# waiwera/waiwera

Measured on AMD Instinct MI355X. Metric: Newton steps/sec, 10M-cell eos_we (BCSR SpMV GB/s in roofline), higher is better.
Workload: dtype f64

## Files before the change

waiwera_amd/csrc/context.hpp:

```cpp
#pragma once
#include <hip/hip_runtime.h>
#include <string>
#include <type_traits>
#include <vector>
#include "../../include/waiwera_hip.h"
#include "colour_order.hpp"
#include "coupling_batch.hpp"
#include "devbuf.hpp"
#include "ilu_schedule.hpp"
#include "mesh_pattern.hpp"
#include "network_pass.hpp"
#include "network_wave.hpp"
#include "physics.hip.h"
#include "tile_schedule.hpp"

namespace wai {

__host__ __device__ __forceinline__ size_t ell_ld(size_t n) {
  size_t ld = (n + 511) & ~(size_t)511;
  if ((ld & 262143) == 0) ld += 512;
  return ld;
}
__host__ __device__ __forceinline__ size_t ell_rows(int bs, size_t n) {
  if (bs >= 3) return ell_ld(n);
  return n;
}
__host__ __device__ __forceinline__ size_t ell_ix1(int bs, size_t n, int r, int k, size_t i) {
  if (bs >= 3) return ((i >> 6) * (size_t)(bs * bs) + (size_t)(r * bs + k)) * 64 + (i & 63);
  return ((size_t)r * n + i) * bs + k;
}
__host__ __device__ __forceinline__ size_t ell_ix(int bs, size_t n, int s, int r, int k, size_t i) {
  if (bs >= 3) {
    const size_t bb = (size_t)(bs * bs);
    return (size_t)(s >> 3) * 8 * bb * ell_ld(n) + ((((i >> 6) << 3) + (size_t)(s & 7)) * bb + (size_t)(r * bs + k)) * 64 + (i & 63);
  }
  return ((size_t)(s * bs + r) * n + i) * bs + k;
}
__host__ __device__ __forceinline__ size_t ell_size(int bs, size_t n, int W) {
  if (bs >= 3) return (size_t)((W + 7) / 8) * 8 * bs * bs * ell_ld(n);
  return (size_t)W * bs * bs * ell_rows(bs, n);
}

enum KClass { KC_EOS = 0, KC_RESIDUAL = 1, KC_JACOBIAN = 2, KC_SPMV = 3, KC_PC_APPLY = 4,
              KC_PC_SETUP = 5, KC_VECTOR = 6, KC_TRANSITIONS = 7, KC_COUNT = 8 };

enum { S_RHO = 0, S_RHOOLD = 1, S_ALPHA = 2, S_OMEGA = 3, S_BETA = 4, S_D1 = 5, S_D2 = 6,
       S_DP2 = 7, S_RHONEW = 8, S_W2 = 9, S_BREAK = 15, S_H = 16 };

enum PcDot { PC_DOT_NONE = 0, PC_DOT_ZA = 1, PC_DOT_XZ = 2, PC_DOT_ZZ = 3, PC_DOT_MERGED = 4 };
static_assert(S_D2 == S_D1 + 1 && S_DP2 == S_D1 + 2 && S_RHONEW == S_D1 + 3 && S_W2 == S_D1 + 4,
              "the merged reductions' slots S_D1 .. S_W2 are consecutive: a reduction addresses them as slot0 + index");
__host__ __device__ constexpr int pc_dot_slot0(int mode) { return mode == PC_DOT_ZZ ? S_DP2 : S_D1; }
__host__ __device__ constexpr int pc_dot_nslots(int mode) {
  return mode == PC_DOT_MERGED ? 5 : (mode == PC_DOT_XZ ? 2 : (mode == PC_DOT_NONE ? 0 : 1));
}

struct Comm;

struct DeviceMesh {
  int n_owned = 0, n_halo = 0, n_bc = 0, n_prim = 0, n_local = 0, n_faces = 0, max_deg = 0;
  DevBuf<double> rock;
  DevBuf<double> vol;
  DevBuf<double> fgeom;
  DevBuf<int> fdir;
  DevBuf<int> adj_face;
  DevBuf<int> adj_other;
  DevBuf<int> adj_blk;
  DevBuf<int> adj_tblk;
  DevBuf<int> diag_blk;
  DevBuf<int> cell_src;
  DevBuf<int> face_cells;
};

struct Sources {
  int n = 0;
  DevBuf<int> cell, comp, pcomp, next;
  DevBuf<double> rate, enth;
  DevBuf<SrcCtl> ctl;
  DevBuf<double> net;
};

struct NetNode { double rate = 0, enth = 0, wrate = 0, wenth = 0, srate = 0, senth = 0; };
struct NetRef { int kind = 0, index = -1; };
struct NetGroup {
  std::vector<NetRef> in;
  int scaling = 0;
  int n_limit = 0, limit_type[3] = {0, 0, 0};
  double limit[3] = {0, 0, 0};
  SrcCtl sep{};
  NetNode node;
};
struct NetOutput {
  int flow = 1;
  NetRef out;
  double rate = -1.0, proportion = -1.0, enthalpy = -1.0;
  NetNode node;
};
struct NetReinjector {
  NetRef in;
  std::vector<NetOutput> out;
  NetRef overflow;
  NetNode node;
  double in_w = 0, in_wh = 0, in_s = 0, in_sh = 0;
  double out_w = 0, out_s = 0;
  NetNode over;
  bool fed = false;
};
struct Network {
  bool on = false;
  std::vector<NetGroup> groups;
  std::vector<NetReinjector> reinjectors;
  std::vector<int> reinj_order;
  std::vector<int> rate_specified, enth_specified;
  std::vector<NetNode> src;
  std::vector<double> h_enth0, h_raw, out_rate, out_enth;
  std::vector<char> is_out;
  std::vector<SrcCtl> h_ctl;
  DevBuf<double> d_raw;
  std::vector<int> gidx;
  int n_global = 0;
  DevBuf<double> d_all;
  std::vector<double> h_loc, l_net, l_enth;
  std::vector<int> h_cell;
  bool coupling = true;
  bool cp_in_pc = true;
  bool cp_valid = false;
  std::vector<int> cp_cells;
  std::vector<double> h_cp_val;
  bool cp_span = false;
  int cp_m = 0, cp_j0 = 0;
  std::vector<int> cp_owner;
  DevBuf<int> d_cp_cells;
  DevBuf<double> d_cp_val, d_cp_f, d_cp_g;
  DevBuf<double> d_cp_x;
  NetFlatHost flat;
  bool flat_fits = false, flat_dirty = true;
  DevBuf<int> d_flat_iw;
  NetWaveHost wave;
  bool wave_built = false, wave_ok = false;
  std::string wave_err;
  DevBuf<int> d_wave_ww;
  DevBuf<double> d_flat_dw;
  DevBuf<double> d_state;
  bool state_on_device = false;
  bool enth_stale = false;
  DevBuf<double> d_cp_yh;
  DevBuf<int> d_cp_flag;
  bool cp_on_device = false;
  DevBuf<double> d_cb_scratch;
  long long cb_doubles = 0;
};

struct Bcsr {
  int n = 0, ncols = 0, nnzb = 0, bs = 0, W = 0;
  int* col = nullptr;
  double* val = nullptr;
  int* rowptr = nullptr;
  int dg = 0;
  double* fdg = nullptr;
};
struct Pattern {
  int n = 0, ncols = 0, nnzb = 0, W = 0;
  DevBuf<int> col;
  DevBuf<int> rowptr;
  std::vector<int> h_rowptr, h_colidx;
};

struct LinSys;
struct TileTables : TileFacts {
  DevBuf<int> tile_ptr;
  DevBuf<int> tile_nin;
  DevBuf<int> ord_f, ord_b;
  DevBuf<int> row_lev;
  void clear() {
    static_cast<TileFacts&>(*this) = TileFacts();
    tile_ptr.reset(); tile_nin.reset(); ord_f.reset(); ord_b.reset(); row_lev.reset();
  }
};
struct IluSchedule : ScheduleFacts {
  DevBuf<int> sub_ptr;
  DevBuf<int> sub_nlev;
  DevBuf<int> sub_split;
  DevBuf<int> row_info;
  DevBuf<unsigned long long> row_infow;
  DevBuf<double> fval;
  DevBuf<double> dinv;
  DevBuf<int> row_uoff;
  DevBuf<int> row_tslot;
  DevBuf<int> sub_int;
  DevBuf<int> sub_bnd;
  DevBuf<int> sub_order;
  DevBuf<int> row_uoffw;
  DevBuf<unsigned short> col16;
  DevBuf<int> sub_seg;
  DevBuf<int> t_info, t_uoff;
  DevBuf<unsigned short> t_col16;
  DevBuf<int> sub_desc;
  DevBuf<int> pack_tab[3];
  DevBuf<int> ord_f;
  DevBuf<int> ord_b;
  TileTables tiles;
  const LinSys* owner = nullptr;
};
struct ColourSchedule : ColourFacts {
  bool built = false;
  bool fused = false;
  DevBuf<int> sub_ptr;
  DevBuf<int> sub_ncol;
  DevBuf<int> rows;
  DevBuf<unsigned long long> slots;
  DevBuf<int> counts;
};
inline int pc_threads(const IluSchedule& s) { return ((s.max_rows + 63) / 64) * 64; }

template <class F>
int with_bs(int bs, F&& f) {
  switch (bs) {
    case 1: f(std::integral_constant<int, 1>{}); return 0;
    case 2: f(std::integral_constant<int, 2>{}); return 0;
    case 3: f(std::integral_constant<int, 3>{}); return 0;
    case 4: f(std::integral_constant<int, 4>{}); return 0;
    default: return -1;
  }
}
template <class F>
void with_flag(bool flag, F&& f) {
  if (flag) f(std::true_type{});
  else f(std::false_type{});
}
template <class F>
int with_eos(int kind, F&& f) {
  switch (kind) {
    case EOS_W: f(std::integral_constant<int, EOS_W>{}); return 0;
    case EOS_WE: f(std::integral_constant<int, EOS_WE>{}); return 0;
    case EOS_WCE: f(std::integral_constant<int, EOS_WCE>{}); return 0;
    case EOS_WSE: f(std::integral_constant<int, EOS_WSE>{}); return 0;
    case EOS_WAE: f(std::integral_constant<int, EOS_WAE>{}); return 0;
    case EOS_WSCE: f(std::integral_constant<int, EOS_WSCE>{}); return 0;
    case EOS_WSAE: f(std::integral_constant<int, EOS_WSAE>{}); return 0;
    default: return -1;
  }
}
struct EosTraits { int np, df, nmob; bool salt; };
inline int eos_traits(int kind, EosTraits& t) {
  return with_eos(kind, [&](auto k) {
    constexpr int K = decltype(k)::value;
    t = EosTraits{EosT<K>::np, EosT<K>::df, EosT<K>::nmob, is_salt<K>};
  });
}

struct AsmSystem {
  int overlap = -1;
  int levels = 0;
  bool sublu = false;
  bool fused = false, fuse_asked = false;
  int n_ext = 0;
  Bcsr E;
  DevBuf<int> E_col;
  DevBuf<double> E_val;
  IluSchedule sched;
  DevBuf<int> ext_row;
  DevBuf<int> gmap;
  DevBuf<double> r_ext;
  bool with_net = false;
  int n_net = 0;
  DevBuf<int> net_pos;
  DevBuf<int> net_pair;
  bool cross = false;
  DevBuf<double> hval;
  DevBuf<double> r_full;
};

struct ResForm {
  int method = 0;
  double dt = 0.0, ratio = 0.0;
  const double* last = nullptr;
  const double* last2 = nullptr;
};

constexpr int MAX_TRACERS = 8;
constexpr int POST_OFF = 64;
constexpr unsigned long long POST_KEY = 0x5bd1e995a5a5c3c3ull;
struct Tracers {
  int nt = 0;
  int phase[MAX_TRACERS] = {0};
  double decay[MAX_TRACERS] = {0}, activation[MAX_TRACERS] = {0}, diffusion[MAX_TRACERS] = {0};
  double* bc = nullptr;
  double* inj = nullptr;
  double* rhsb = nullptr;
  int mode = 0;
  long long n_sweeps = 0;
  unsigned char kernarg_tail[136] = {0};
};
static_assert(sizeof(Tracers) == 408, "Tracers is a kernel argument (k_tracer_assemble_all, k_tracer_lhs): its size is part of their argument layout");
static_assert(std::is_trivially_copyable<Tracers>::value, "a kernel argument holds views, never an owner");

struct TracerForm {
  int method, it, nt, phase;
  double dt, ratio, decay, activation, diffusion;
};
static_assert(std::is_trivially_copyable<TracerForm>::value && std::is_trivially_copyable<ResForm>::value &&
              std::is_trivially_copyable<EosParams>::value, "a kernel argument holds views, never an owner");

constexpr int FIN_MAXF = 64;
struct Fin {
  int count = 0;
  int nb = 0;
  int nf = 1;
  double* part2 = nullptr;
  int slot0 = 0, nslots = 0;
  int phase = -1;
  int seq = 0;
  double* scal = nullptr;
  double* post = nullptr;
};
static_assert(std::is_trivially_copyable<Fin>::value, "a kernel argument holds views, never an owner");

struct Krylov {
  double* d_post = nullptr;
  int seq = 0;
  long long n_launch = 0, n_copy = 0;
  DevBuf<double> partials;
  DevBuf<double> partials2;
  DevBuf<unsigned> started;
  bool alpha_pending = false;
  int nb_max = 0;
  DevBuf<double> scal;
  PinnedBuf<double> h_scal;
  int nblocks = 0;
  int nb_pc = 0;
};

struct KrylovVecs {
  DevBuf<double> R, RP, P, V, S, T, tmp, X_own;
  double* X = nullptr;
  DevBuf<double> bl;
  DevBuf<double> basis;
  int basis_m = 0;
};

struct KspOpts {
  int type = WAI_KSP_BCGS, restart = 30, max_its = 10000;
  double rtol = 1.e-5, atol = 1.e-50;
};
struct PcOpts {
  int type = WAI_AUX_PC_FOLLOW, asm_overlap = 1, ilu_levels = 0, sub = WAI_SUB_ILU;
};

struct LinSys {
  Bcsr A;
  DevBuf<double> val, fdg;
  KspOpts ksp;
  PcOpts pc;
  int n = 0, nl = 0;
  KrylovVecs* kv = nullptr;
  AsmSystem as;
  bool net_blocks = false;
};

struct Gather {
  DevBuf<double> in;
  DevBuf<double> send;
  DevBuf<double> recv;
  DevBuf<double> out;
  DevBuf<double> counts;
  DevBuf<int> idx;
  DevBuf<int> claim;
  DevBuf<int> flag;
  size_t n_in = 0, n_send = 0, n_recv = 0, n_out = 0, n_counts = 0, n_idx = 0, n_claim = 0;
};

}

namespace wai {
struct LuBlocks {
  DevBuf<double> inv;
  DevBuf<size_t> inv_ptr;
  std::vector<size_t> h_inv_ptr;
  size_t total = 0;
  int bs = 0;
};
int launch_lu_apply(wai_ctx* c, int bs, const double* r, double* z);

struct Handles {
  hipStream_t stream = nullptr;
  Comm* comm = nullptr;
  hipEvent_t ev_scal = nullptr;
  hipStream_t comm_stream = nullptr;
  hipEvent_t ev_pack = nullptr, ev_halo = nullptr;
  hipEvent_t ev0 = nullptr, ev1 = nullptr, pev0 = nullptr, pev1 = nullptr;
  Handles() = default;
  Handles(const Handles&) = delete;
  ~Handles();
};
}

struct wai_ctx : wai::Handles {
  int device = 0;
  int n_cu = 256;
  size_t lds_per_block = 64 * 1024;
  int kind = 0, np = 0, df = 0, nmob = 0;
  bool salt = false;
  wai::EosParams ep{};
  wai_solver_opts opts{};
  int sub_pc = WAI_SUB_ILU;
  int net_pass = WAI_NETWORK_PASS_HOST;
  int net_walk = WAI_NETWORK_WALK_LANE;
  int net_wave_attr = 0;
  long long net_passes = 0, net_waits = 0;
  int cp_build = WAI_COUPLING_BUILD_COLUMNS;
  long long cp_launches = 0, cp_columns = 0, cp_chunks = 0;
  int pc_ordering = WAI_PC_ORDER_NATURAL;
  wai::ColourSchedule colour;
  std::vector<int> pc_tiles;
  wai::DeviceMesh mesh;
  wai::Sources src;
  wai::Network net;
  std::vector<int> src_gidx;
  int src_nglobal = 0;
  wai::Pattern pat;
  wai::LinSys flow, aux, coupled;
  wai::KrylovVecs kv, kv_coupled;
  wai::IluSchedule ilu;
  wai::LuBlocks lu;
  wai::Krylov ks;
  wai::Tracers tr;
  wai::Gather gat;
  wai::DevBuf<double> tr_bc, tr_inj, tr_rhsb;
  wai::DevBuf<double> flu, flu_last_iter, flu_last_step, flu_pert;
  wai::DevBuf<double> hstep;
  wai::DevBuf<double> w_y, w_yold, w_delta, w_f, w_lhs, w_a, w_b, w_c;
  wai::DevBuf<int> d_flags;
  wai::PinnedBuf<int> h_flags;
  wai::DevBuf<double> d_red;
  wai::PinnedBuf<double> h_red;
  wai::DevBuf<double> stage[4];
  size_t stage_len = 0;
  struct EnvSw {
    bool fin_separate = false; bool no_col16 = false; bool scalar_kernels = false; bool iluk_level_path = false;
    bool asm_unfused = false; bool no_desc_share = false; bool no_pack = false;
    bool colour_sweeps = false;
    int park_stage = -1;
  } env;
  int test_drop_wait = 0;
  int n_nbr = 0;
  std::vector<int> nbr_rank, send_ptr, recv_ptr;
  wai::DevBuf<int> d_send_idx; wai::DevBuf<double> d_sendbuf, d_recvbuf;
  int send_total = 0, max_dof_buf = 0;
  double fnorm0 = 0.0;
  int method = 0;
  double ratio = 0.0;
  wai::DevBuf<double> w_lhs2;
  int scheme = 0, taken = 0;
  double dt_last = 0.0;
  wai::DevBuf<double> w_hist;
  wai::DevBuf<double> w_hist_prev;
  double dt_last_prev = 0.0;
  bool can_reject = false;
  bool prof_on = false;
  bool last_iter_partial = false;
  double prof_ms[wai::KC_COUNT] = {0};
  long long prof_n[wai::KC_COUNT] = {0};
  std::string err;
  bool bc_set = false;
  int dbg = 0;
};

namespace wai {
int launch_eos(wai_ctx* c, const double* y, int first, int count, bool perturbed);
int launch_residual(wai_ctx* c, double dt, const double* lhs_old, double* f, double* lhs_out,
                    double* rhs_out, const int* only = nullptr, int n_only = 0);
int launch_jacobian(wai_ctx* c, double dt, const double* lhs_old);
int launch_transitions(wai_ctx* c, const double* y_old, double* search, double* y);
int launch_tracer_assemble(wai_ctx* c, const TracerForm& tf, const double* alx_last,
                           const double* alx_last2, double* b);
int launch_tracer_assemble_all(wai_ctx* c, int method, double dt, double ratio, const double* alx_last,
                               const double* alx_last2, double* b);
int launch_tracer_lhs(wai_ctx* c, double* Al);
int launch_separator(wai_ctx* c, double pressure, double* out);
int launch_face_fluxes(wai_ctx* c, const int* face_cells, double* out);
int launch_source_rates(wai_ctx* c, double* out, bool raw = false);
int launch_network_pass(wai_ctx* c, const double* raw, double* net, double* enth, double* state_out, bool wave);
int net_wave_allow_lds(wai_ctx* c, const void* kernel, int bit, size_t* bytes);
int launch_cp_perturb(wai_ctx* c, double* p, double* yh);
int launch_cp_restore(wai_ctx* c, double* p, const double* yh);
int launch_cp_diff(wai_ctx* c, int ml, int m, int bs, int j, int k, const double* g, const double* yh, double* val, int* flag);
int launch_coupling_batch(wai_ctx* c, const CouplingBatch& b, int col0, int ncol, double dt, const double* y, const double* lhs_old,
                          long long* launches, bool wave);
int launch_tracer_pick(wai_ctx* c, const double* X, int it, double* x);
int launch_tracer_put(wai_ctx* c, const double* x, int it, double* X);
int launch_tracer_alx(wai_ctx* c, const double* X, double* alx);
int launch_max_scaled(wai_ctx* c, const double* v, const double* scale, double tol, double* val,
                      int* idx);
int launch_fluid_aos(wai_ctx* c, const double* flu_soa, double* out_aos);
int launch_region_get(wai_ctx* c, double* out);
int launch_region_set(wai_ctx* c, const double* in, int first, int count);

int launch_spmv(wai_ctx* c, const Bcsr& M, const double* x, double* y);
int launch_ilu_factor_on(wai_ctx* c, const Bcsr& M, IluSchedule& s);
int launch_pc_on(wai_ctx* c, const Bcsr& M, const IluSchedule& s, bool spmv, const double* in, double* z,
                 int dot_mode, const double* aux, const int* list = nullptr, int nrun = 0, const Fin* fin = nullptr,
                 const double* in2 = nullptr, const Bcsr* F = nullptr, const int* row_map = nullptr);
int pc_kernel_kind(const wai_ctx* c, const Bcsr& M, const IluSchedule& s);
bool pc_axpy_capable(const wai_ctx* c, const Bcsr& M);
bool pc_axpy_default(const wai_ctx* c, const Bcsr& M);
int launch_big_solve(wai_ctx* c, const Bcsr& M, const IluSchedule& s, double* z);
int launch_colour_factor(wai_ctx* c, const Bcsr& M, const ColourSchedule& k, IluSchedule& s);
int launch_colour_solve(wai_ctx* c, const Bcsr& M, const ColourSchedule& k, const IluSchedule& s, double* z);
bool pc_colour_serves(const wai_ctx* c, const Bcsr& M, const ColourSchedule& k, bool one_rank);
int launch_pc_colour(wai_ctx* c, const Bcsr& M, const ColourSchedule& k, const IluSchedule& s, bool spmv, const double* in, double* z,
                     int dot_mode, const double* aux, const Fin* fin = nullptr);
int launch_sublu_solve(wai_ctx* c, const Bcsr& M, const IluSchedule& s, double* z);
bool sublu_vector_in_lds(const IluSchedule& s, int bs);
int launch_asm_gather_matrix(wai_ctx* c, const Bcsr& M, const AsmSystem& a);
int launch_pack_rows(wai_ctx* c, const Bcsr& M);
int launch_unpack_rows(wai_ctx* c, const Bcsr& M, const AsmSystem& a);
int launch_asm_gather(wai_ctx* c, const AsmSystem& a, const double* r);
int launch_asm_scatter(wai_ctx* c, const AsmSystem& a, double* z);
int vec_dots(wai_ctx* c, const double* a1, const double* b1, int slot1, const double* a2, const double* b2,
             int slot2, int n);
int launch_pc(wai_ctx* c, const Bcsr& M, bool spmv, const double* in, double* z, int dot_mode, const double* aux,
              const int* list = nullptr, int nrun = 0, const Fin* fin = nullptr, const double* in2 = nullptr);
Fin make_fin(wai_ctx* c, int slot0, int nslots, int phase, bool post = false);
inline Fin make_fin_dots(wai_ctx* c, int dot_mode, int phase, bool post = false) {
  return make_fin(c, pc_dot_slot0(dot_mode), pc_dot_nslots(dot_mode), phase, post);
}
int launch_ell_to_bcsr(wai_ctx* c, const Bcsr& M, double* bcsr);
int launch_dg_spmv(wai_ctx* c, const Bcsr& M, const double* x, double* y);
int launch_dg_factor(wai_ctx* c, const Bcsr& M, IluSchedule& s);
int launch_dg_pc(wai_ctx* c, const Bcsr& M, const IluSchedule& s, bool spmv, const double* in, double* z, const int* list, int nrun);
int launch_dg_big_solve(wai_ctx* c, const Bcsr& M, const IluSchedule& s, double* z);
int launch_dg_to_bcsr(wai_ctx* c, const Bcsr& M, double* bcsr);
int launch_bcsr_to_ell(wai_ctx* c, const double* bcsr, const Bcsr& M);
int vec_finalize(wai_ctx* c, int nb, int slot0, int nslots, int phase);
int vec_dot(wai_ctx* c, const double* a, const double* b, int n, int slot);
int partials_clear(wai_ctx* c, int slot0, int nslots);
int vec_copy(wai_ctx* c, double* dst, const double* src, size_t n);
int vec_zero(wai_ctx* c, double* dst, size_t n);
int vec_waxpy(wai_ctx* c, double* w, double alpha, const double* x, const double* y, int n);
int bcgs_scalars(wai_ctx* c, int phase, bool post = false);
int bcgs_update_xrp_derive(wai_ctx* c, const KrylovVecs& k, int n);
int bcgs_post(wai_ctx* c, int seq);
void read_env(wai_ctx* c);
int test_drop_partials(wai_ctx* c, int n);
int bcgs_update_p(wai_ctx* c, const KrylovVecs& k, int n);
int bcgs_update_s(wai_ctx* c, const KrylovVecs& k, int n);
int bcgs_update_xr(wai_ctx* c, const KrylovVecs& k, int n, bool dots = true, int fin_phase = -2, bool post = false);
int bcgs_update_xrp(wai_ctx* c, const KrylovVecs& k, int n);
int pack_halo_axpy(wai_ctx* c, const double* a, const double* b, int dof, hipStream_t stream = nullptr);
int gmres_mdot(wai_ctx* c, const double* basis, size_t ld, int n, const double* w, int k);
int gmres_maxpy_norm(wai_ctx* c, const double* basis, size_t ld, int n, double* w, int k);
int gmres_scale_to(wai_ctx* c, double* dst, const double* src, int slot_norm2, int n);
int gmres_update_x(wai_ctx* c, const double* basis, size_t ld, int n, double* x, const double* ycoef_host, int k);
int pack_halo(wai_ctx* c, const double* vec, int dof, hipStream_t stream = nullptr);
int unpack_halo(wai_ctx* c, double* vec, int dof, hipStream_t stream = nullptr);
}
```

waiwera_amd/csrc/linalg_device.hip.h:

```cpp
#pragma once
#include "context.hpp"

namespace wai {

constexpr int TPB = 256;

template <int CTRL, int ROW_MASK, int BANK_MASK>
__device__ __forceinline__ double dpp_add(double v) {
  const int lo = __builtin_amdgcn_update_dpp(0, __double2loint(v), CTRL, ROW_MASK, BANK_MASK, false);
  const int hi = __builtin_amdgcn_update_dpp(0, __double2hiint(v), CTRL, ROW_MASK, BANK_MASK, false);
  return v + __hiloint2double(hi, lo);
}
__device__ __forceinline__ double wave_sum(double v) {
#ifdef WAI_SHFL_SUMS
  for (int off = 32; off > 0; off >>= 1) v += __shfl_down(v, off);
  return __shfl(v, 0);
#else
  v = dpp_add<0x111, 0xf, 0xf>(v);
  v = dpp_add<0x112, 0xf, 0xf>(v);
  v = dpp_add<0x114, 0xf, 0xe>(v);
  v = dpp_add<0x118, 0xf, 0xc>(v);
  v = dpp_add<0x142, 0xa, 0xf>(v);
  v = dpp_add<0x143, 0xc, 0xf>(v);
  return __hiloint2double(__builtin_amdgcn_readlane(__double2hiint(v), 63), __builtin_amdgcn_readlane(__double2loint(v), 63));
#endif
}
constexpr int WMAX = 8;
constexpr int WMAX_WIDE = MAX_CELL_FACES;


__device__ __forceinline__ int xcd_remap(int b, int n) {
  const int per = (n + 7) >> 3;
  return (b & 7) * per + (b >> 3);
}

template <int BS>
__device__ __forceinline__ size_t vix(int n, int s, int e, int i) {
  return ell_ix(BS, (size_t)n, s, e / BS, e % BS, (size_t)i);
}
template <int BS>
__device__ __forceinline__ size_t dix(int n, int e, int i) {
  return ell_ix1(BS, (size_t)n, e / BS, e % BS, (size_t)i);
}
typedef double wai_d2 __attribute__((ext_vector_type(2)));
__device__ __forceinline__ int load_col(const int* __restrict__ col, size_t idx) {
  return __builtin_nontemporal_load(col + idx);
}
__device__ __forceinline__ void store_z2(double* __restrict__ z, size_t i, double a, double b) {
  wai_d2 v = {a, b};
  __builtin_nontemporal_store(v, reinterpret_cast<wai_d2*>(z + i * 2));
}
template <int BS>
__device__ __forceinline__ void load_block(const double* __restrict__ val, int n, int s, int i, double* b) {
  if constexpr (BS == 2) {
    const size_t i0 = ell_ix(2, (size_t)n, s, 0, 0, (size_t)i), i1 = ell_ix(2, (size_t)n, s, 1, 0, (size_t)i);
    const wai_d2 r0 = __builtin_nontemporal_load(reinterpret_cast<const wai_d2*>(val + i0));
    const wai_d2 r1 = __builtin_nontemporal_load(reinterpret_cast<const wai_d2*>(val + i1));
    b[0] = r0.x; b[1] = r0.y; b[2] = r1.x; b[3] = r1.y;
  } else {
#pragma unroll
    for (int e = 0; e < BS * BS; e++) b[e] = val[vix<BS>(n, s, e, i)];
  }
}

template <int BS>
__device__ __forceinline__ void load_pivot(const double* __restrict__ val, int n, int i, double* b) {
  if constexpr (BS <= 2) load_block<BS>(val, n, 0, i, b);
  else {
#pragma unroll
    for (int e = 0; e < BS * BS; e++) b[e] = val[dix<BS>(n, e, i)];
  }
}

typedef double wai_d2u __attribute__((ext_vector_type(2), aligned(8)));
template <int BS>
__device__ __forceinline__ void load_x(const double* __restrict__ x, int col, double* xv) {
  if constexpr (BS == 2) {
    const double2 t = *reinterpret_cast<const double2*>(x + (size_t)col * 2);
    xv[0] = t.x; xv[1] = t.y;
  } else if constexpr (BS == 3) {
    const double* p = x + (size_t)col * 3;
    const wai_d2u t = *reinterpret_cast<const wai_d2u*>(p);
    xv[0] = t.x; xv[1] = t.y; xv[2] = p[2];
  } else if constexpr (BS == 4) {
    const double* p = x + (size_t)col * 4;
    const wai_d2u t = *reinterpret_cast<const wai_d2u*>(p), u = *reinterpret_cast<const wai_d2u*>(p + 2);
    xv[0] = t.x; xv[1] = t.y; xv[2] = u.x; xv[3] = u.y;
  } else {
#pragma unroll
    for (int k = 0; k < BS; k++) xv[k] = x[(size_t)col * BS + k];
  }
}

template <int BS, bool AX>
__device__ __forceinline__ void load_xs(const double* __restrict__ in, const double* __restrict__ in2, double nalpha,
                                        int col, double* xv) {
  load_x<BS>(in, col, xv);
  if constexpr (AX) {
    double x2[BS];
    load_x<BS>(in2, col, x2);
#pragma unroll
    for (int k = 0; k < BS; k++) xv[k] = __builtin_fma(nalpha, x2[k], xv[k]);
  }
}

template <int BS>
__device__ __forceinline__ void load_x_stream(const double* __restrict__ x, int col, double* xv) {
  if constexpr (BS == 2) {
    const wai_d2 t = __builtin_nontemporal_load(reinterpret_cast<const wai_d2*>(x + (size_t)col * 2));
    xv[0] = t.x; xv[1] = t.y;
  } else {
#pragma unroll
    for (int k = 0; k < BS; k++) xv[k] = x[(size_t)col * BS + k];
  }
}

template <int BS, int WM = WMAX>
__device__ __forceinline__ void ell_row_mult(int n, int W, int i, const int* __restrict__ col,
                                             const double* __restrict__ val,
                                             const double* __restrict__ x, double* acc) {
  constexpr int BB = BS * BS;
  int cs[WM];
#pragma unroll
  for (int s = 0; s < WM; s++) {
    cs[s] = i;
    if (s < W) cs[s] = load_col(col, (size_t)s * n + i);
  }
#pragma unroll
  for (int s = 0; s < WM; s++) {
    if (s < W) {
      const int c = cs[s];
      double xv[BS], a[BS * BS];
      load_x<BS>(x, c, xv);
      load_block<BS>(val, n, s, i, a);
#pragma unroll
      for (int r = 0; r < BS; r++)
#pragma unroll
        for (int k = 0; k < BS; k++) acc[r] += a[r * BS + k] * xv[k];
    }
  }
}

template <int BS>
__device__ __forceinline__ bool block_inverse(const double* a, double* inv) {
  double m[BS][2 * BS];
#pragma unroll
  for (int r = 0; r < BS; r++)
#pragma unroll
    for (int c = 0; c < BS; c++) { m[r][c] = a[r * BS + c]; m[r][BS + c] = (r == c) ? 1.0 : 0.0; }
  bool ok = true;
#pragma unroll
  for (int p = 0; p < BS; p++) {
    int piv = p;
#pragma unroll
    for (int r = p + 1; r < BS; r++)
      if (fabs(m[r][p]) > fabs(m[piv][p])) piv = r;
#pragma unroll
    for (int r = p + 1; r < BS; r++)
      if (r == piv) {
#pragma unroll
        for (int c = 0; c < 2 * BS; c++) { const double t = m[p][c]; m[p][c] = m[r][c]; m[r][c] = t; }
      }
    if (m[p][p] == 0.0) ok = false;
    const double d = 1.0 / m[p][p];
#pragma unroll
    for (int c = 0; c < 2 * BS; c++) m[p][c] *= d;
#pragma unroll
    for (int r = 0; r < BS; r++)
      if (r != p) {
        const double f = m[r][p];
#pragma unroll
        for (int c = 0; c < 2 * BS; c++) m[r][c] -= f * m[p][c];
      }
  }
#pragma unroll
  for (int r = 0; r < BS; r++)
#pragma unroll
    for (int c = 0; c < BS; c++) inv[r * BS + c] = m[r][BS + c];
  return ok;
}

__device__ __forceinline__ void unpack_info(int info, int& lfirst, int& dslot, int& ulast, int& lf,
                                            int& lb) {
  lfirst = info & 15; dslot = (info >> 4) & 15; ulast = (info >> 8) & 15;
  lf = (info >> 12) & 1023; lb = (info >> 22) & 1023;
}

__device__ __forceinline__ void unpack_info_wide(int info, int& lfirst, int& dslot, int& ulast) {
  lfirst = info & 255; dslot = (info >> 8) & 255; ulast = (info >> 16) & 255;
}

__device__ __forceinline__ void unpack_info_w(unsigned long long info, int& lfirst, int& dslot, int& ulast, int& lf,
                                              int& lb) {
  const unsigned w0 = (unsigned)info, w1 = (unsigned)(info >> 32);
  lfirst = w0 & 31; dslot = (w0 >> 5) & 31; ulast = (w0 >> 10) & 31;
  lf = w1 & 1023; lb = (w1 >> 10) & 1023;
}

}
```

waiwera_amd/csrc/pc_park.hip.h:

```cpp
#pragma once
#include "reductions.hip.h"

namespace wai {

template <bool SPMV, bool AX, bool C16, bool PACK = false, bool STAGE = false>
__global__ __launch_bounds__(512, 6) void k_pc_park(
    int n, int W, int nsub, const int* __restrict__ sub_ptr, const int* __restrict__ sub_nlev,
    const int* __restrict__ sub_desc, const int* __restrict__ row_info, const int* __restrict__ row_uoff, const int* __restrict__ col,
    const unsigned short* __restrict__ col16, const int* __restrict__ sub_seg,
    const double* __restrict__ sval, const double* __restrict__ dinv, const double* __restrict__ in,
    const double* __restrict__ in2, const double* __restrict__ scal,
    double* __restrict__ z, const double* __restrict__ aux, double* partials, int nb_max, int dot,
    const int* __restrict__ sub_list, Fin fin, Stagger stagger) {
  constexpr int BS = 2, BB = 4, MLU = 3;
  static_assert(!STAGE || (SPMV && C16), "the staged operand is the operator's, on the 16-bit column indices");
  extern __shared__ __attribute__((aligned(16))) double lds[];
  if (fin_block(fin, partials, nb_max)) return;
  int s = xcd_remap(blockIdx.x, nsub);
  if (s >= nsub) return;
  int toff = 0, ubase = 0, nl_grp = 0;
  if constexpr (PACK) {
    const int w = __builtin_amdgcn_readfirstlane((int)threadIdx.x >> 6);
    const int4 rec = reinterpret_cast<const int4*>(sub_list)[(size_t)s * 8 + w];
    s = rec.x; toff = rec.y; ubase = rec.z; nl_grp = rec.w;
  } else {
    if (sub_list) s = sub_list[s];
  }
  const bool member = !PACK || s >= 0;
  const int lo = member ? sub_ptr[s] : 0, R = member ? sub_ptr[s + 1] - lo : 0;
  int dlo = lo;
  if constexpr (C16) dlo = member ? sub_desc[s] : 0;
  const int nl = PACK ? nl_grp : sub_nlev[s];
  const int nlf = nl & 0xffff, nlb = nl >> 16;
  const int tid = threadIdx.x, lob = lo - toff, i = lob + tid, di = dlo - toff + tid;
  const bool active = tid - toff < R;
  const double nalpha = AX ? -scal[S_ALPHA] : 0.0;
  stagger_start(stagger);
  double* ys = lds;
  double* upark = lds + (size_t)blockDim.x * BS + 80 + (size_t)ubase * BB;
  double Lf[MLU][BB];
  int Lc[MLU], Uc[MLU], lf = -1, lb = -1, uo = 0, nU = 0;
  double xin[BS] = {0.0, 0.0}, avp[BS] = {0.0, 0.0};
#pragma unroll
  for (int p = 0; p < MLU; p++) {
    Lc[p] = tid; Uc[p] = tid;
#pragma unroll
    for (int e = 0; e < BB; e++) Lf[p][e] = 0.0;
  }
  int lfirst = 0, dslot = 0, ulast = 0;
  int cgs[WMAX];
  [[maybe_unused]] double own2[BS], blk0[BB], xr0[BS], xv0[BS];
  [[maybe_unused]] bool far0 = false;
  if (active) {
    unpack_info(row_info[di], lfirst, dslot, ulast, lf, lb);
    uo = row_uoff[di];
    nU = ulast - dslot - 1;
    if constexpr (STAGE) {
      load_x<BS>(in, i, xin);
      if constexpr (AX) load_x<BS>(in2, i, own2);
    }
    if constexpr (C16) {
      const int* sg = sub_seg + (size_t)s * 8;
      const int g0 = sg[0], g1 = sg[1], g2 = sg[2], g3 = sg[3], g4 = sg[4], g5 = sg[5], g6 = sg[6], g7 = sg[7];
      typedef unsigned wai_u4v __attribute__((ext_vector_type(4)));
      const wai_u4v pk = reinterpret_cast<const wai_u4v*>(col16)[di];
      const unsigned pw[4] = {pk.x, pk.y, pk.z, pk.w};
      unsigned cu[WMAX];
#pragma unroll
      for (int q = 0; q < WMAX; q++) cu[q] = (pw[q >> 1] >> (16 * (q & 1))) & 0xffffu;
#pragma unroll
      for (int q = 0; q < WMAX; q++) {
        const unsigned code = cu[q] >> 13;
        int b = g0;
        b = code == 1 ? g1 : b; b = code == 2 ? g2 : b; b = code == 3 ? g3 : b; b = code == 4 ? g4 : b;
        b = code == 5 ? g5 : b; b = code == 6 ? g6 : b; b = code == 7 ? g7 : b;
        cgs[q] = q < W ? b + (int)(cu[q] & 8191u) : i;
      }
    } else {
#pragma unroll
      for (int q = 0; q < WMAX; q++) {
        cgs[q] = i;
        if (q < W) cgs[q] = load_col(col, (size_t)q * n + i);
      }
    }
    if constexpr (STAGE) {
      load_block<BS>(sval, n, 0, i, blk0);
      if constexpr (AX) {
#pragma unroll
        for (int k = 0; k < BS; k++) xin[k] = __builtin_fma(nalpha, own2[k], xin[k]);
      }
      *reinterpret_cast<double2*>(ys + tid * 2) = make_double2(xin[0], xin[1]);
      far0 = lfirst > 0;
      if (far0) {
        load_x<BS>(in, cgs[0], xr0);
        if constexpr (AX) load_x<BS>(in2, cgs[0], xv0);
      }
    }
  }
  if constexpr (STAGE) {
    lds_barrier();
    __builtin_amdgcn_s_waitcnt(0x0f70);
  }
  double acc[BS] = {0.0, 0.0};
  if (active) {
#pragma unroll
    for (int q = 0; q < WMAX; q++) {
      if (q < W) {
        const int cg = cgs[q];
        double blk[BB];
        if constexpr (STAGE) {
          if (q == 0) {
#pragma unroll
            for (int e = 0; e < BB; e++) blk[e] = blk0[e];
          } else load_block<BS>(sval, n, q, i, blk);
          const bool inb = (q >= lfirst) && (q < ulast);
          const double2 sv = *reinterpret_cast<const double2*>(ys + ((inb && q != dslot) ? cg - lob : tid) * 2);
          double xv[BS] = {q == dslot ? xin[0] : sv.x, q == dslot ? xin[1] : sv.y};
          if (!inb) {
            if (q == 0) {
              asm volatile("" : "+v"(xr0[0]), "+v"(xr0[1]));
              xv[0] = xr0[0]; xv[1] = xr0[1];
              if constexpr (AX) { xv[0] = __builtin_fma(nalpha, xv0[0], xv[0]); xv[1] = __builtin_fma(nalpha, xv0[1], xv[1]); }
            } else load_xs<BS, AX>(in, in2, nalpha, cg, xv);
          }
          acc[0] += blk[0] * xv[0] + blk[1] * xv[1];
          acc[1] += blk[2] * xv[0] + blk[3] * xv[1];
        } else load_block<BS>(sval, n, q, i, blk);
        if constexpr (SPMV && !STAGE) {
          double xv[BS];
          load_xs<BS, AX>(in, in2, nalpha, cg, xv);
          acc[0] += blk[0] * xv[0] + blk[1] * xv[1];
          acc[1] += blk[2] * xv[0] + blk[3] * xv[1];
          xin[0] = q == dslot ? xv[0] : xin[0];
          xin[1] = q == dslot ? xv[1] : xin[1];
        }
        const bool isl = (q >= lfirst) && (q < dslot), isu = (q > dslot) && (q < ulast);
#pragma unroll
        for (int p = 0; p < MLU; p++) {
          const bool tl = isl && (q - lfirst == p), tu = isu && (q - dslot - 1 == p);
          Lc[p] = tl ? cg - lob : Lc[p];
          Uc[p] = tu ? cg - lob : Uc[p];
#pragma unroll
          for (int e = 0; e < BB; e++) Lf[p][e] = tl ? blk[e] : Lf[p][e];
        }
        if (isu) {
          double* dst = upark + (size_t)(uo + (q - dslot - 1)) * BB;
          *reinterpret_cast<double2*>(dst) = make_double2(blk[0], blk[1]);
          *reinterpret_cast<double2*>(dst + 2) = make_double2(blk[2], blk[3]);
        }
      }
    }
    if constexpr (!SPMV) {
      double r[BS], dv[BB];
      load_x<BS>(in, i, r);
      load_pivot<BS>(dinv, n, i, dv);
      acc[0] = dv[0] * r[0] + dv[1] * r[1];
      acc[1] = dv[2] * r[0] + dv[3] * r[1];
      xin[0] = r[0]; xin[1] = r[1];
    }
    if (dot == PC_DOT_ZA || dot == PC_DOT_MERGED) load_x_stream<BS>(aux, i, avp);
  }
  if constexpr (STAGE) lds_barrier();
  if (active) *reinterpret_cast<double2*>(ys + tid * 2) = make_double2(acc[0], acc[1]);
  __syncthreads();
  auto gather3 = [&](const int (&cc)[MLU], const double (&ff)[MLU][BB], double* sum) {
    double2 yk[MLU];
#pragma unroll
    for (int p = 0; p < MLU; p++) yk[p] = *reinterpret_cast<const double2*>(ys + cc[p] * 2);
#pragma unroll
    for (int r = 0; r < BS; r++) {
      double part[MLU];
#pragma unroll
      for (int p = 0; p < MLU; p++) part[p] = ff[p][r * BS] * yk[p].x + ff[p][r * BS + 1] * yk[p].y;
      sum[r] = (part[0] + part[1]) + part[2];
    }
  };
  for (int lev = 1; lev < nlf; lev++) {
    if (lf == lev) {
      const double2 a = *reinterpret_cast<const double2*>(ys + tid * 2);
      double sum[BS];
      gather3(Lc, Lf, sum);
      *reinterpret_cast<double2*>(ys + tid * 2) = make_double2(a.x - sum[0], a.y - sum[1]);
    }
    __syncthreads();
  }
#pragma unroll
  for (int p = 0; p < MLU; p++) {
    const bool have = p < nU;
    const double* src = upark + (size_t)(uo + (have ? p : 0)) * BB;
    const double2 u0 = *reinterpret_cast<const double2*>(src), u1 = *reinterpret_cast<const double2*>(src + 2);
    Lf[p][0] = have ? u0.x : 0.0; Lf[p][1] = have ? u0.y : 0.0;
    Lf[p][2] = have ? u1.x : 0.0; Lf[p][3] = have ? u1.y : 0.0;
  }
  double out[BS] = {0.0, 0.0};
  for (int lev = 0; lev < nlb; lev++) {
    if (lb == lev) {
      const double2 a = *reinterpret_cast<const double2*>(ys + tid * 2);
      double sum[BS];
      gather3(Uc, Lf, sum);
      out[0] = a.x - sum[0];
      out[1] = a.y - sum[1];
      *reinterpret_cast<double2*>(ys + tid * 2) = make_double2(out[0], out[1]);
    }
    if (lev + 1 < nlb) __syncthreads();
  }
  if (active) store_z2(z, (size_t)i, out[0], out[1]);
  if (dot != 0) {
    double* red = lds + (size_t)blockDim.x * BS;
    double v[5] = {0.0, 0.0, 0.0, 0.0, 0.0};
    if constexpr (STAGE) {
      auto hi = [](const double (&p)[BS], const double (&r)[BS]) { return __builtin_fma(p[0], r[0], p[1] * r[1]); };
      auto lo = [](const double (&p)[BS], const double (&r)[BS]) { return __builtin_fma(p[1], r[1], p[0] * r[0]); };
      if (dot == PC_DOT_ZA) {
        if (active) v[0] = hi(out, avp);
      } else if (dot == PC_DOT_XZ) {
        v[0] = hi(xin, out); v[1] = hi(out, out);
      } else if (dot == PC_DOT_MERGED) {
        if (active) { v[0] = hi(xin, out); v[1] = hi(out, out); v[2] = lo(xin, xin); v[3] = lo(xin, avp); v[4] = hi(out, avp); }
      } else {
        v[0] = hi(out, out);
      }
    } else
    pc_row_dots<BS, true, false>(dot, v, out, active, [&](double (&x)[BS]) { x[0] = xin[0]; x[1] = xin[1]; },
                                 [&](double (&a)[BS]) { a[0] = avp[0]; a[1] = avp[1]; });
    __syncthreads();
    if constexpr (PACK) pc_reduce_dots_waves(dot, v, red, partials, nb_max, s, toff >> 6, (R + 63) >> 6);
    else pc_reduce_dots(dot, v, red, partials, nb_max, s);
  }
}

}
```

Baseline: 5.551.

## Slice the 2x2-block ELL value layout into 64-row groups of eight slots

```diff
diff --git a/waiwera_amd/csrc/context.hpp b/waiwera_amd/csrc/context.hpp
--- a/waiwera_amd/csrc/context.hpp
+++ b/waiwera_amd/csrc/context.hpp
@@ -7,6 +7,7 @@
 #include "colour_order.hpp"
 #include "coupling_batch.hpp"
 #include "devbuf.hpp"
+#include "ell_layout.hpp"
 #include "ilu_schedule.hpp"
 #include "mesh_pattern.hpp"
 #include "network_pass.hpp"
@@ -16,30 +17,6 @@
 
 namespace wai {
 
-__host__ __device__ __forceinline__ size_t ell_ld(size_t n) {
-  size_t ld = (n + 511) & ~(size_t)511;
-  if ((ld & 262143) == 0) ld += 512;
-  return ld;
-}
-__host__ __device__ __forceinline__ size_t ell_rows(int bs, size_t n) {
-  if (bs >= 3) return ell_ld(n);
-  return n;
-}
-__host__ __device__ __forceinline__ size_t ell_ix1(int bs, size_t n, int r, int k, size_t i) {
-  if (bs >= 3) return ((i >> 6) * (size_t)(bs * bs) + (size_t)(r * bs + k)) * 64 + (i & 63);
-  return ((size_t)r * n + i) * bs + k;
-}
-__host__ __device__ __forceinline__ size_t ell_ix(int bs, size_t n, int s, int r, int k, size_t i) {
-  if (bs >= 3) {
-    const size_t bb = (size_t)(bs * bs);
-    return (size_t)(s >> 3) * 8 * bb * ell_ld(n) + ((((i >> 6) << 3) + (size_t)(s & 7)) * bb + (size_t)(r * bs + k)) * 64 + (i & 63);
-  }
-  return ((size_t)(s * bs + r) * n + i) * bs + k;
-}
-__host__ __device__ __forceinline__ size_t ell_size(int bs, size_t n, int W) {
-  if (bs >= 3) return (size_t)((W + 7) / 8) * 8 * bs * bs * ell_ld(n);
-  return (size_t)W * bs * bs * ell_rows(bs, n);
-}
 
 enum KClass { KC_EOS = 0, KC_RESIDUAL = 1, KC_JACOBIAN = 2, KC_SPMV = 3, KC_PC_APPLY = 4,
               KC_PC_SETUP = 5, KC_VECTOR = 6, KC_TRANSITIONS = 7, KC_COUNT = 8 };
diff --git a/waiwera_amd/csrc/ell_layout.hpp b/waiwera_amd/csrc/ell_layout.hpp
--- /dev/null
+++ b/waiwera_amd/csrc/ell_layout.hpp
@@ -0,0 +1,47 @@
+#pragma once
+#include <cstddef>
+
+#if defined(__HIPCC__)
+#include <hip/hip_runtime.h>
+#define WAI_ELL_FN __host__ __device__ __forceinline__
+#else
+#define WAI_ELL_FN inline
+#endif
+
+namespace wai {
+
+WAI_ELL_FN size_t ell_ld(size_t n) {
+  size_t ld = (n + 511) & ~(size_t)511;
+  if ((ld & 262143) == 0) ld += 512;
+  return ld;
+}
+WAI_ELL_FN size_t ell_rows(int bs, size_t n) {
+  if (bs >= 3) return ell_ld(n);
+  return n;
+}
+WAI_ELL_FN bool ell_sliced(int bs) {
+#ifdef WAI_ELL_PLANES
+  return bs >= 3;
+#else
+  return bs >= 2;
+#endif
+}
+WAI_ELL_FN size_t ell_ix1(int bs, size_t n, int r, int k, size_t i) {
+  if (bs >= 3) return ((i >> 6) * (size_t)(bs * bs) + (size_t)(r * bs + k)) * 64 + (i & 63);
+  return ((size_t)r * n + i) * bs + k;
+}
+WAI_ELL_FN size_t ell_ix(int bs, size_t n, int s, int r, int k, size_t i) {
+  if (bs >= 3) {
+    const size_t bb = (size_t)(bs * bs);
+    return (size_t)(s >> 3) * 8 * bb * ell_ld(n) + ((((i >> 6) << 3) + (size_t)(s & 7)) * bb + (size_t)(r * bs + k)) * 64 + (i & 63);
+  }
+  if (bs == 2 && ell_sliced(2))
+    return (size_t)(s >> 3) * 32 * ell_ld(n) + ((((i >> 6) << 3) + (size_t)(s & 7)) * 2 + (size_t)r) * 128 + (i & 63) * 2 + (size_t)k;
+  return ((size_t)(s * bs + r) * n + i) * bs + k;
+}
+WAI_ELL_FN size_t ell_size(int bs, size_t n, int W) {
+  if (ell_sliced(bs)) return (size_t)((W + 7) / 8) * 8 * bs * bs * ell_ld(n);
+  return (size_t)W * bs * bs * n;
+}
+
+}
diff --git a/waiwera_amd/csrc/linalg_device.hip.h b/waiwera_amd/csrc/linalg_device.hip.h
--- a/waiwera_amd/csrc/linalg_device.hip.h
+++ b/waiwera_amd/csrc/linalg_device.hip.h
@@ -64,9 +64,27 @@
 }
 
 template <int BS>
+__device__ __forceinline__ const double* row_base(const double* __restrict__ val, int n, int i) {
+  if constexpr (BS == 2) {
+    if (ell_sliced(2)) return val + (size_t)i * 2 + (size_t)(i >> 6) * 1920;
+  }
+  return val + ell_ix(BS, (size_t)n, 0, 0, 0, (size_t)i);
+}
+template <int BS>
+__device__ __forceinline__ void load_block_row(const double* __restrict__ rowp, int n, int s, double* b) {
+  static_assert(BS == 2, "the 16-byte block rows of 2 x 2 blocks");
+  const wai_d2 r0 = __builtin_nontemporal_load(reinterpret_cast<const wai_d2*>(rowp + ell_ix(2, (size_t)n, s, 0, 0, 0)));
+  const wai_d2 r1 = __builtin_nontemporal_load(reinterpret_cast<const wai_d2*>(rowp + ell_ix(2, (size_t)n, s, 1, 0, 0)));
+  b[0] = r0.x; b[1] = r0.y; b[2] = r1.x; b[3] = r1.y;
+}
+
+template <int BS>
 __device__ __forceinline__ void load_pivot(const double* __restrict__ val, int n, int i, double* b) {
-  if constexpr (BS <= 2) load_block<BS>(val, n, 0, i, b);
-  else {
+  if constexpr (BS == 2) {
+    const wai_d2 r0 = __builtin_nontemporal_load(reinterpret_cast<const wai_d2*>(val + dix<2>(n, 0, i)));
+    const wai_d2 r1 = __builtin_nontemporal_load(reinterpret_cast<const wai_d2*>(val + dix<2>(n, 2, i)));
+    b[0] = r0.x; b[1] = r0.y; b[2] = r1.x; b[3] = r1.y;
+  } else {
 #pragma unroll
     for (int e = 0; e < BS * BS; e++) b[e] = val[dix<BS>(n, e, i)];
   }
@@ -121,6 +139,8 @@
                                              const double* __restrict__ x, double* acc) {
   constexpr int BB = BS * BS;
   int cs[WM];
+  [[maybe_unused]] const double* rowp = nullptr;
+  if constexpr (BS == 2) rowp = row_base<BS>(val, n, i);
 #pragma unroll
   for (int s = 0; s < WM; s++) {
     cs[s] = i;
@@ -132,7 +152,8 @@
       const int c = cs[s];
       double xv[BS], a[BS * BS];
       load_x<BS>(x, c, xv);
-      load_block<BS>(val, n, s, i, a);
+      if constexpr (BS == 2) load_block_row<BS>(rowp, n, s, a);
+      else load_block<BS>(val, n, s, i, a);
 #pragma unroll
       for (int r = 0; r < BS; r++)
 #pragma unroll
diff --git a/waiwera_amd/csrc/pc_park.hip.h b/waiwera_amd/csrc/pc_park.hip.h
--- a/waiwera_amd/csrc/pc_park.hip.h
+++ b/waiwera_amd/csrc/pc_park.hip.h
@@ -51,7 +51,9 @@
   int cgs[WMAX];
   [[maybe_unused]] double own2[BS], blk0[BB], xr0[BS], xv0[BS];
   [[maybe_unused]] bool far0 = false;
+  const double* rowp = sval;
   if (active) {
+    rowp = row_base<BS>(sval, n, i);
     unpack_info(row_info[di], lfirst, dslot, ulast, lf, lb);
     uo = row_uoff[di];
     nU = ulast - dslot - 1;
@@ -84,7 +86,7 @@
       }
     }
     if constexpr (STAGE) {
-      load_block<BS>(sval, n, 0, i, blk0);
+      load_block_row<BS>(rowp, n, 0, blk0);
       if constexpr (AX) {
 #pragma unroll
         for (int k = 0; k < BS; k++) xin[k] = __builtin_fma(nalpha, own2[k], xin[k]);
@@ -112,7 +114,7 @@
           if (q == 0) {
 #pragma unroll
             for (int e = 0; e < BB; e++) blk[e] = blk0[e];
-          } else load_block<BS>(sval, n, q, i, blk);
+          } else load_block_row<BS>(rowp, n, q, blk);
           const bool inb = (q >= lfirst) && (q < ulast);
           const double2 sv = *reinterpret_cast<const double2*>(ys + ((inb && q != dslot) ? cg - lob : tid) * 2);
           double xv[BS] = {q == dslot ? xin[0] : sv.x, q == dslot ? xin[1] : sv.y};
@@ -125,7 +127,7 @@
           }
           acc[0] += blk[0] * xv[0] + blk[1] * xv[1];
           acc[1] += blk[2] * xv[0] + blk[3] * xv[1];
-        } else load_block<BS>(sval, n, q, i, blk);
+        } else load_block_row<BS>(rowp, n, q, blk);
         if constexpr (SPMV && !STAGE) {
           double xv[BS];
           load_xs<BS, AX>(in, in2, nalpha, cg, xv);
```

Measured after the change: 5.518. Within noise of the previous version (-0.6%).
